# dlwns147/amq

Measured on AMD Instinct MI355X. Metric: decode tokens/s, Llama-2-7B AMQ mixed 2/3/4-bit avg-3-bit, batch 1, higher is better.
Workload: dtype f16; 1 GPU; Llama-2-7B shapes, synthesized avg-3.0-bit per-layer arch (bits_usage 2.982), batch 1 decode after a 64-token prefill, one stream per GPU; parallelism=replicas x1, prompt=64, group_size=128

## Files before the change

amq_amd/_lib.py:

```python
import ctypes
import os

_HERE = os.path.dirname(os.path.abspath(__file__))
LIB_PATH = os.path.join(_HERE, "libamq_hip.so")
AB_LIB_PATH = os.path.join(_HERE, "libamq_hip_ab.so")

AMQ_OK = 0
MODE_HQQ, MODE_FMA, MODE_FMA1 = 0, 1, 2
PRO_NONE, PRO_RMSNORM, PRO_SILU_MUL = 0, 1, 2
PRO_MUL = 4
MAX_SEGMENTS = 4
MATH_DEFAULT, MATH_LINEAR, MATH_GROUPSCALE, MATH_EXACT = 0, 1, 2, 3
FEWROW_AUTO, FEWROW_TILE, FEWROW_STREAM = 0, 1, 2
ABI_VERSION = 521
LOOKUP_STATE_WORDS = 32
STEP_STATE_STRIDE = 272
GEMM_AUTO, GEMM_TILED, GEMM_SKINNY, GEMM_RING, GEMM_RING128, GEMM_WS, GEMM_DEQ = 0, 1, 2, 3, 4, 5, 6
HQQ_ITERS = 20
HQQ_INFO_BYTES = 88
GPTQ_INFO_BYTES = 4
AWQ_INFO_BYTES = 4
OWQ_INFO_BYTES = 4
AWQ_STEPS = 10

_vp, _i, _f, _sz = ctypes.c_void_p, ctypes.c_int, ctypes.c_float, ctypes.c_size_t


class Segment(ctypes.Structure):
    _fields_ = [("qweight_native", _vp), ("meta_native", _vp), ("bias", _vp), ("residual", _vp),
                ("y", _vp), ("N", _i), ("bits", _i), ("mode", _i), ("y_stride", _i)]


class EngineLinear(ctypes.Structure):
    _fields_ = [("qweight_native", _vp), ("meta_native", _vp), ("N", _i), ("bits", _i), ("mode", _i), ("reserved", _i)]
# ... 77 lines not shown
    "amq_attn_prefill_xfrag_f16": (_i, [_vp, _vp, _vp, _vp, _i, _i, _i, _i, _i] + [ctypes.c_longlong] * 5 + [_vp]),
    "amq_gemv_f16w_rows": (_i, [_vp, _vp, _vp, _vp, _vp, _f, _i, _i, _i, _vp]),
    "amq_decode_tail_batch_f16": (_i, [_vp, _i, _vp, _i, _vp, _vp, _vp, _vp, _vp, _i, _i, _vp]),
    "amq_decode_tail_suppress_f16": (_i, [_vp, _i, _vp, _i, _vp, _vp, _vp, _vp, _vp, _i, _i, _vp, _vp]),
    "amq_sample_f16": (_i, [_vp, _i, _i, _vp, _vp, _vp, _vp, _vp, _i, _i, _vp]),
    "amq_decode_tail_sample_f16": (_i, [_vp, _i, _vp, _i, _vp, _vp, _vp, _vp, _vp, _i, _i, _vp, _vp, _vp]),
    "amq_logit_nll_f16": (_i, [_vp, ctypes.c_longlong, _vp, _i, _i, _vp, _vp, _vp, _vp]),
    "amq_logit_jsd_f16": (_i, [_vp, ctypes.c_longlong, _vp, ctypes.c_longlong, _i, _i, _i, _f, _vp, _vp]),
    "amq_set_token_f16": (_i, [_vp, _i, _vp, _i, _i, _vp, _vp, _vp, _vp, _vp, _i, _i, _vp]),
    "amq_attn_decode_seq_f16": (_i, [_vp, _vp, _vp, _vp, _vp, _vp, _vp, _i, _i, _i, _i, _i, _i, _vp, _sz, _vp, _vp]),
    "amq_decode_tail_seq_f16": (_i, [_vp, _i, _vp, _i, _vp, _vp, _vp, _vp, _i, _i, _vp, _vp]),
    "amq_decode_tail_sample_seq_f16": (_i, [_vp, _i, _vp, _i, _vp, _vp, _vp, _vp, _i, _i, _vp, _vp, _vp]),
    "amq_set_token_seq_f16": (_i, [_vp, _i, _vp, _i, _i, _vp, _vp, _vp, _vp, _i, _i, _vp]),
    "amq_attn_decode_rows_f16": (_i, [_vp, _vp, _vp, _vp, _vp, _vp, _vp, _i, _i, _i, _i, _i, _i, _vp, _sz, _vp, _vp]),
    "amq_attn_decode_rows_gqa_f16": (_i, [_vp, _vp, _vp, _vp, _vp, _vp, _vp, _i, _i, _i, _i, _i, _i, _vp, _sz, _vp, _vp]),
    "amq_decode_tail_lookup_f16": (_i, [_vp, _i, _vp, _i, _vp, _vp, _vp, _vp, _i, _i, _vp, _vp, _vp, _i, _vp]),
    "amq_decode_tail_lookup_sample_f16": (_i, [_vp, _i, _vp, _i, _vp, _vp, _vp, _vp, _i, _i, _vp, _vp, _vp, _i, _vp, _vp, _vp, _vp]),
    "amq_attn_prefill_f16": (_i, [_vp, _vp, _vp, _vp, _i, _i, _i, _i, _i, _i] + [ctypes.c_longlong] * 10 + [_vp]),
    "amq_rope_cache_f16": (_i, [_vp, _vp, _vp, _vp, _vp, _vp, _i, _i, _i, _i, _i, _i, _i, _vp]),
    "amq_rope_cache_batch_f16": (_i, [_vp, _vp, _vp, _vp, _vp, _vp, _i, _i, _i, _i, _i, _i, _i, _i, _vp]),
    "amq_rope_rows_f16": (_i, [_vp, _vp, _vp, _i, _i, _i, _i, _i, _i, _i, _vp]),
    "amq_silu_mul_f16": (_i, [_vp, _vp, _vp, _sz, _vp]),
    "amq_gemv_grouped_f16": (_i, [ctypes.POINTER(Segment), _i, _vp, _vp, _vp, _f, _i, _i, _i, _i, _i, ctypes.POINTER(GemvOpts), _vp]),
    "amq_gemv_grouped_sums_f16": (_i, [ctypes.POINTER(Segment), _i, _vp, _vp, _f, _vp, _vp, _i, _i, _i, _vp]),
    "amq_gemm_f16w_f16": (_i, [_vp, _vp, _vp, _vp, _vp, _vp, _i, _i, _i, _i, _i, _vp]),
    "amq_gemm_route_workspace_bytes": (_sz, [_i, _i, _i, _i]),
    "amq_gemm_route_workspace_bytes_g": (_sz, [_i, _i, _i, _i, _i]),
    "amq_gemm_res_norm_xfrag_f16": (_i, [_i, _i, _vp, _vp, _vp, _vp, _vp, _vp, _i, _i, _i, _i, _i, _vp, _sz, _vp, _f, _vp, _vp]),
    "amq_gemm_route_f16": (_i, [_i, _i, _i, _vp, _vp, _vp, _vp, _vp, _vp, _i, _i, _i, _i, _i, _i, _vp, _sz, _vp]),
}

for _base in ("amq_attn_decode_f16", "amq_attn_decode_cur_f16", "amq_attn_decode_split_f16", "amq_attn_decode_seq_f16", "amq_attn_decode_rows_f16",
              "amq_attn_decode_rows_gqa_f16",
              "amq_rope_cache_batch_f16", "amq_rope_rows_f16"):
    SIGNATURES[_base.replace("_batch", "")[:-len("_f16")] + "_qkn_f16"] = (_i, [_qkn] + SIGNATURES[_base][1])
del _base

AB_SIGNATURES = {
    "amq_gemv_qkv_attn_f16": (_i, [ctypes.POINTER(Segment), _vp, _vp, _f, _i, _i, _vp, _vp, _vp, _vp, _i, _i, _i, _i, _vp, _vp]),
    "amq_decode_engine_image_bytes": (_sz, [_i]),
    "amq_decode_engine_scratch_bytes": (_sz, [_i, _i, _i]),
    "amq_decode_engine_sync_bytes": (_sz, []),
    "amq_decode_engine_image": (_i, [ctypes.POINTER(EngineBlock), _i, _i, _i, _i, _i, _i, _i, _vp]),
    "amq_decode_engine_f16": (_i, [_vp, _i, _i, _i, _i, _i, _i, _i, _f, _vp, _vp, _sz, _vp, _vp, _sz, _i, _vp]),
}

# ... 122 lines not shown
```

amq_amd/csrc/amq_capi.hip:

```cpp
#include "../../include/amq_hip.h"
#ifdef AMQ_AB_ROUTES
#include "../../include/amq_hip_ab.h"
#endif
#include "amq_common.cuh"
#include "amq_kernels.h"

#include <stdarg.h>
#include <stdio.h>
#include <vector>

namespace {

thread_local char g_err[512] = "";

int fail(int code, const char* fmt, ...) {
    va_list ap;
    va_start(ap, fmt);
    vsnprintf(g_err, sizeof(g_err), fmt, ap);
    va_end(ap);
    return code;
}

int check_hip(hipError_t e, const char* what) {
    if (e == hipSuccess) return AMQ_OK;
// ... 268 lines not shown
}

#ifndef AMQ_GEMV_DEFAULT_MATH
#define AMQ_GEMV_DEFAULT_MATH AMQ_MATH_EXACT
#endif
int amq_default_gemv_math(void) { return AMQ_GEMV_DEFAULT_MATH; }

int amq_gemv_grouped_f16(const amq_segment* segs, int nseg, const void* x, const void* x2, const void* gamma,
                         float eps, int prologue, int M, int K, int group, int x_stride, const amq_gemv_opts* opts,
                         void* stream) {
    if (!segs || nseg < 1 || nseg > AMQ_MAX_SEGMENTS) return fail(AMQ_EINVAL, "nseg must be 1..%d (got %d)", AMQ_MAX_SEGMENTS, nseg);
    if (!x) return fail(AMQ_EINVAL, "null x");
    if ((prologue < AMQ_PRO_NONE || prologue > AMQ_PRO_SILU_MUL) && prologue != AMQ_PRO_MUL) return fail(AMQ_EINVAL, "unknown prologue %d", prologue);
    if (prologue == AMQ_PRO_RMSNORM && !gamma) return fail(AMQ_EINVAL, "RMSNorm prologue needs gamma");
    if (prologue == AMQ_PRO_SILU_MUL && !x2) return fail(AMQ_EINVAL, "SiLU*mul prologue needs x2");
    if (prologue == AMQ_PRO_MUL && !x2) return fail(AMQ_EINVAL, "mul prologue needs x2");
    if (M < 1) return fail(AMQ_ESHAPE, "M must be >= 1 (got %d)", M);
    amq_gemv_opts o{};
    if (opts) o = *opts;
    if (o.math < AMQ_MATH_DEFAULT || o.math > AMQ_MATH_EXACT)
        return fail(AMQ_EINVAL, "opts.math must be AMQ_MATH_DEFAULT, AMQ_MATH_EXACT, AMQ_MATH_GROUPSCALE or AMQ_MATH_LINEAR");
    if (o.math == AMQ_MATH_DEFAULT) o.math = amq_default_gemv_math();
    if (o.waves != 0 && o.waves != 4 && o.waves != 8 && o.waves != 16) return fail(AMQ_EINVAL, "opts.waves must be 0, 4, 8 or 16");
    if (o.depth != 0 && o.depth != 2 && o.depth != 4) return fail(AMQ_EINVAL, "opts.depth must be 0, 2 or 4");
    if (o.rpt < 0 || o.rpt > 64) return fail(AMQ_EINVAL, "opts.rpt (row-tiles per workgroup) must be 0..64");
    if (o.act_mask < 0 || o.act_mask >= (1 << nseg)) return fail(AMQ_EINVAL, "opts.act_mask names segments 0..%d (got 0x%x)", nseg - 1, o.act_mask);
    if ((o.act_mask || prologue == AMQ_PRO_MUL) && amq::meta_pairs(group) != 1)
        return fail(AMQ_ESHAPE, "opts.act_mask / AMQ_PRO_MUL: groups of 128 (and multiples) only (got %d); use AMQ_PRO_SILU_MUL", group);
    const bool plain_form = !o.dot && o.math != AMQ_MATH_LINEAR && o.depth != 4 && amq::meta_pairs(group) == 1 && o.waves != 4;
    const bool whole_rows = prologue == AMQ_PRO_RMSNORM || (x_stride != 0 && x_stride != K);
    if (M > amq::GEMV_MAX_M || amq::gemv_min_lds_bytes(M, K, plain_form && o.waves == 0 && o.rpt == 0, whole_rows) > LDS_LIMIT)
        return fail(AMQ_ESHAPE, "M=%d rows of K=%d%s do not fit LDS for the GEMV path; use amq_gemm_f16", M, K, (x_stride != 0 && x_stride != K) ? " (strided x)" : "");
    amq::GemvArgs a{};
    for (int i = 0; i < nseg; ++i) {
        const amq_segment& s = segs[i];
        if (int rc = check_shape(s.bits, s.N, K, group)) return rc;
        if (int rc = check_mode(s.mode)) return rc;
        if (!s.qweight_native || !s.meta_native || !s.y) return fail(AMQ_EINVAL, "segment %d: null pointer", i);
        amq::GemvSeg& d = a.seg[i];
        d.qweight = s.qweight_native; d.meta = s.meta_native; d.bias = s.bias; d.residual = s.residual; d.y = s.y;
        d.N = s.N; d.bits = s.bits; d.mode = s.mode;
        d.y_stride = s.y_stride ? s.y_stride : s.N;
        d.act = (o.act_mask >> i) & 1;
        if (d.act && s.residual) return fail(AMQ_EINVAL, "segment %d: an activated output (opts.act_mask) takes no residual", i);
    }
    a.nseg = nseg; a.M = M; a.K = K; a.x_stride = x_stride ? x_stride : K;
    a.x = x; a.x2 = x2; a.gamma = gamma; a.eps = eps; a.prologue = prologue;
    a.flags = (o.dot ? amq::GEMV_FLAG_DOT : 0) | (o.math == AMQ_MATH_LINEAR ? amq::GEMV_FLAG_LINEAR : 0) |
              (o.math == AMQ_MATH_GROUPSCALE ? amq::GEMV_FLAG_GS : 0);
    a.force_waves = o.waves;
    a.force_depth = o.depth;
    a.force_rpt = o.rpt;
    a.gp = amq::meta_pairs(group);
    if (a.gp > 1 && (o.dot || o.math == AMQ_MATH_LINEAR || o.depth == 4))
        return fail(AMQ_EINVAL, "groups of %d: the GEMV kernel's default form only (opts.math = AMQ_MATH_EXACT, opts.dot = 0, opts.depth = 0 / 2)", group);
    return check_hip(amq::launch_gemv(a, (hipStream_t)stream), "gemv");
}

int amq_gemv_grouped_sums_f16(const amq_segment* segs, int nseg, const void* x, const void* gamma, float eps, const float* sums_in,
                              float* sums_out, int M, int K, int group, void* stream) {
    if (!segs || nseg < 1 || nseg > AMQ_MAX_SEGMENTS) return fail(AMQ_EINVAL, "nseg must be 1..%d (got %d)", AMQ_MAX_SEGMENTS, nseg);
    if (!x) return fail(AMQ_EINVAL, "null x");
    if ((sums_in != nullptr) != (gamma != nullptr)) return fail(AMQ_EINVAL, "sums_in (the partial sums of squares of x) and gamma go together");
    if (M < 2 || M > 8) return fail(AMQ_ESHAPE, "the partial-sum forms live in the 2 .. 8-row kernels (got M=%d); one row: amq_gemv_grouped_f16 with AMQ_PRO_RMSNORM", M);
    if (amq::meta_pairs(group) != 1) return fail(AMQ_ESHAPE, "groups of 128 (and multiples) only (got %d)", group);
    if (K < 2048) return fail(AMQ_ESHAPE, "K >= 2048 (the 2 .. 8-row kernels run 8 or 16 waves per workgroup; got K=%d)", K);
    if (sums_out && nseg != 1) return fail(AMQ_EINVAL, "sums_out describes ONE output: nseg must be 1");
    if (sums_out && sums_in) return fail(AMQ_EINVAL, "sums_out is written by launches without a prologue (o_proj, down_proj): not together with sums_in");
    if (sums_in && K > 8192) return fail(AMQ_ESHAPE, "sums_in: K <= 8192 (K / 16 <= 512 partials per row; got K=%d)", K);
    const bool phased = amq::gemv_rows_phased(M, K, true, sums_in != nullptr);
    if (sums_in && phased) return fail(AMQ_ESHAPE, "M=%d rows of K=%d are staged in two K phases: no fused norm there", M, K);
    if (amq::gemv_min_lds_bytes(M, K, true, sums_in != nullptr) > LDS_LIMIT)
        return fail(AMQ_ESHAPE, "M=%d rows of K=%d do not fit LDS for the GEMV path", M, K);
    amq::GemvArgs a{};
    for (int i = 0; i < nseg; ++i) {
        const amq_segment& s = segs[i];
        if (int rc = check_shape(s.bits, s.N, K, group)) return rc;
        if (int rc = check_mode(s.mode)) return rc;
        if (!s.qweight_native || !s.meta_native || !s.y) return fail(AMQ_EINVAL, "segment %d: null pointer", i);
// ... 915 lines not shown
```

amq_amd/csrc/amq_gemv.hip:

```cpp
#include "amq_gemv_body.cuh"

namespace amq {


#ifdef AMQ_STAMP
unsigned long long* g_stamp_ptr = nullptr;
extern "C" int amq_debug_set_stamps(void* p) { g_stamp_ptr = (unsigned long long*)p; return 0; }
#endif

size_t gemv_lds_bytes(int M, int K, int nw) {
    const size_t xbytes = (((size_t)M * (K + XPAD) * 2) + 15) & ~(size_t)15;
    const size_t xg = (size_t)(K >> 7) * 64;
    const size_t red = (size_t)2 * (nw > 1 ? nw : 16) * 16 * 16 * 4;
    return xbytes + xg + red;
}

size_t gemv_lds_bytes_rows(int M, int K, int nw) {
    const size_t xbytes = (((size_t)M * (K + XPAD) * 2) + 15) & ~(size_t)15;
    return xbytes + (size_t)2 * nw * (M <= 4 ? 64 : 128) * 4;
}
bool gemv_rows_phased(int M, int K, bool plain, bool norm) {
    const int G = K >> 7;
    return plain && !norm && M > 4 && M <= 8 && (G & 1) == 0 && G / 2 >= 2 * 16 && (K / 2 >> 3) <= 1024 &&
           gemv_lds_bytes_rows(M, K, 16) > 160 * 1024 && gemv_lds_bytes_rows(M, K / 2, 16) <= 160 * 1024;
// ... 2 lines not shown
    if (gemv_rows_phased(M, K, plain, norm)) return gemv_lds_bytes_rows(M, K / 2, 16);
    if (plain && M > 1 && M <= 8) return gemv_lds_bytes_rows(M, K, 16);
    return gemv_lds_bytes(M, K, 1);
}

int gemv_pick_waves(int total_rt, int K) {
    const int G = K >> 7;
    if (G < 16) return 4;
    if (G > 32) return 16;
    return 8;
}

#define AMQ_GEMV_EXTERN(PRO_)                                                                                                  \
    extern template hipError_t launch_pro<PRO_>(const GemvKArgs&, int, int, int, int, size_t, hipStream_t);                     \
    extern template hipError_t launch_pro_g<PRO_, 2>(const GemvKArgs&, int, int, size_t, hipStream_t);                          \
    extern template hipError_t launch_pro_g<PRO_, 4>(const GemvKArgs&, int, int, size_t, hipStream_t);
AMQ_GEMV_EXTERN(PRO_NONE)
AMQ_GEMV_EXTERN(PRO_RMSNORM)
AMQ_GEMV_EXTERN(PRO_SILU_MUL)
#undef AMQ_GEMV_EXTERN
extern template hipError_t launch_pro<PRO_MUL>(const GemvKArgs&, int, int, int, int, size_t, hipStream_t);
hipError_t launch_pro_sums_entry(const GemvKArgs&, int nw, int rs, int, size_t, hipStream_t);

#ifndef AMQ_RS128_THREE
#define AMQ_RS128_THREE 1
#endif
hipError_t launch_gemv(GemvArgs& a, hipStream_t st) {
    StreamDevice sd_(st);
    int total_rt = 0;
    for (int i = 0; i < a.nseg; ++i) { a.seg[i].n_rt = a.seg[i].N / 16; total_rt += a.seg[i].n_rt; }
    int nw = a.force_waves ? a.force_waves : gemv_pick_waves(total_rt, a.K);
    const int gp = a.gp > 1 ? a.gp : 1;
    if (gp != 1 && gp != 2 && gp != 4) return hipErrorInvalidValue;
    if (gp > 1 && ((a.flags & (GEMV_FLAG_DOT | GEMV_FLAG_LINEAR)) || a.force_depth == 4)) return hipErrorInvalidValue;
    bool rs128 = false, rs64 = false;
    const bool plain = !(a.flags & (GEMV_FLAG_DOT | GEMV_FLAG_LINEAR)) && a.force_depth != 4 && gp == 1;
    const bool ph2 = !a.force_waves && a.force_rpt <= 0 && gemv_rows_phased(a.M, a.K, plain, a.prologue == PRO_RMSNORM || a.x_stride != a.K);
    if (ph2) {
        rs128 = true;
        nw = 16;
    } else if (a.M > 1 && a.M <= 8 && plain && nw != 4) {
        rs128 = a.M > 4;
        rs64 = !rs128;
        if (!a.force_waves && nw == 8 && 2 * gemv_lds_bytes_rows(a.M, a.K, 8) > 160 * 1024) nw = 16;
    } else if (!a.force_waves && a.M > 1 && nw == 8 && 3 * gemv_lds_bytes(a.M, a.K, 8) > 160 * 1024) {
        nw = 16;
    }
    const bool mid_k = gp == 1 && !a.force_waves && nw == 16 && a.M == 1 && (a.K >> 3) > 512 && (a.K >> 3) <= 1024 &&
                       !(a.flags & (GEMV_FLAG_DOT | GEMV_FLAG_LINEAR)) && a.force_depth != 4;
    if (mid_k) nw = 8;
    int rpt = ph2 ? 1 : a.force_rpt;
// ... 40 lines not shown
        k.wg_begin[i] = s.wg_begin; k.n_rt[i] = gemv_split(s.n_rt, s.wg_count); k.key[i] = s.bits * 4 + (s.mode == MODE_FMA1 && !has_fma1 ? (int)MODE_FMA : s.mode);
        k.qweight[i] = s.qweight; k.meta[i] = s.meta;
        k.bias[i] = s.bias; k.residual[i] = s.residual; k.y[i] = s.y; k.y_stride[i] = s.y_stride;
        k.act_mask |= (s.act ? 1 : 0) << i;
    }
#ifdef AMQ_STAMP
    k.stamps = g_stamp_ptr;
#endif
    if (gp == 2) {
        switch (a.prologue) {
            case PRO_NONE: return launch_pro_g<PRO_NONE, 2>(k, nw, wg, lds, st);
            case PRO_RMSNORM: return launch_pro_g<PRO_RMSNORM, 2>(k, nw, wg, lds, st);
            default: return launch_pro_g<PRO_SILU_MUL, 2>(k, nw, wg, lds, st);
        }
    }
    if (gp == 4) {
        switch (a.prologue) {
            case PRO_NONE: return launch_pro_g<PRO_NONE, 4>(k, nw, wg, lds, st);
            case PRO_RMSNORM: return launch_pro_g<PRO_RMSNORM, 4>(k, nw, wg, lds, st);
            default: return launch_pro_g<PRO_SILU_MUL, 4>(k, nw, wg, lds, st);
        }
    }
    if (a.prologue == PRO_RMSNORM_SUMS) return launch_pro_sums_entry(k, nw, rs64 ? 64 : 128, wg, lds, st);
    switch (a.prologue) {
        case PRO_NONE: return launch_pro<PRO_NONE>(k, a.flags | (rs128 ? GEMV_FLAG_RS128 : 0) | (rs64 ? GEMV_FLAG_RS64 : 0) | (ph2 ? GEMV_FLAG_PH2 : 0), a.force_depth, nw, wg, lds, st);
        case PRO_RMSNORM: return launch_pro<PRO_RMSNORM>(k, a.flags | (rs128 ? GEMV_FLAG_RS128 : 0) | (rs64 ? GEMV_FLAG_RS64 : 0) | (ph2 ? GEMV_FLAG_PH2 : 0), a.force_depth, nw, wg, lds, st);
        case PRO_MUL: return launch_pro<PRO_MUL>(k, a.flags | (rs128 ? GEMV_FLAG_RS128 : 0) | (rs64 ? GEMV_FLAG_RS64 : 0) | (ph2 ? GEMV_FLAG_PH2 : 0), a.force_depth, nw, wg, lds, st);
        default: return launch_pro<PRO_SILU_MUL>(k, a.flags | (rs128 ? GEMV_FLAG_RS128 : 0) | (rs64 ? GEMV_FLAG_RS64 : 0) | (ph2 ? GEMV_FLAG_PH2 : 0), a.force_depth, nw, wg, lds, st);
    }
}

}
```

amq_amd/csrc/amq_gemv_body.cuh:

```cuda
#pragma once
#include "amq_common.cuh"
#include "amq_kernels.h"

namespace amq {

constexpr int XPAD = 8;

struct GemvKArgs {
    const void* x; const void* x2; const void* gamma;
    int M, K, x_stride, nseg;
    float eps; int rpt, pad0_, pad1_;
    int wg_begin[GEMV_MAX_SEG];
    int n_rt[GEMV_MAX_SEG];
    int key[GEMV_MAX_SEG];
    const void* qweight[GEMV_MAX_SEG];
    const void* meta[GEMV_MAX_SEG];
    const void* bias[GEMV_MAX_SEG];
    const void* residual[GEMV_MAX_SEG];
    void* y[GEMV_MAX_SEG];
    int y_stride[GEMV_MAX_SEG];
    float* sums_out;
    int sums_stride;
    int act_mask;
#ifdef AMQ_STAMP
// ... 845 lines not shown
    const _Float16* xuse = xl;
    constexpr bool HAS_FMA1 = (MATH == MATH_EXACT || MATH == MATH_GS) && GP == 1;
    bool done = false;
    if constexpr (HAS_FMA1) {
        if (key == 4 * 4 + MODE_FMA1) { gemv_body<4, MODE_FMA1, PRO, NW, U, MATH, XCH, RS, false, GP, PH>(a, blk, sidx, qwp, mtp, nrt, local, xl, xuse, xg, red, xs, xmode, xr); done = true; }
        else if (key == 3 * 4 + MODE_FMA1) { gemv_body<3, MODE_FMA1, PRO, NW, U, MATH, XCH, RS, false, GP, PH>(a, blk, sidx, qwp, mtp, nrt, local, xl, xuse, xg, red, xs, xmode, xr); done = true; }
        else if (key == 2 * 4 + MODE_FMA1) { gemv_body<2, MODE_FMA1, PRO, NW, U, MATH, XCH, RS, false, GP, PH>(a, blk, sidx, qwp, mtp, nrt, local, xl, xuse, xg, red, xs, xmode, xr); done = true; }
    }
    if (!done) switch (key) {
        case 4 * 4 + MODE_HQQ: gemv_body<4, MODE_HQQ, PRO, NW, U, MATH, XCH, RS, false, GP, PH>(a, blk, sidx, qwp, mtp, nrt, local, xl, xuse, xg, red, xs, xmode, xr); break;
        case 3 * 4 + MODE_HQQ: gemv_body<3, MODE_HQQ, PRO, NW, U, MATH, XCH, RS, false, GP, PH>(a, blk, sidx, qwp, mtp, nrt, local, xl, xuse, xg, red, xs, xmode, xr); break;
        case 2 * 4 + MODE_HQQ: gemv_body<2, MODE_HQQ, PRO, NW, U, MATH, XCH, RS, false, GP, PH>(a, blk, sidx, qwp, mtp, nrt, local, xl, xuse, xg, red, xs, xmode, xr); break;
        case 4 * 4 + MODE_FMA: gemv_body<4, MODE_FMA, PRO, NW, U, MATH, XCH, RS, false, GP, PH>(a, blk, sidx, qwp, mtp, nrt, local, xl, xuse, xg, red, xs, xmode, xr); break;
        case 3 * 4 + MODE_FMA: gemv_body<3, MODE_FMA, PRO, NW, U, MATH, XCH, RS, false, GP, PH>(a, blk, sidx, qwp, mtp, nrt, local, xl, xuse, xg, red, xs, xmode, xr); break;
        default:               gemv_body<2, MODE_FMA, PRO, NW, U, MATH, XCH, RS, false, GP, PH>(a, blk, sidx, qwp, mtp, nrt, local, xl, xuse, xg, red, xs, xmode, xr); break;
    }
    if (threadIdx.x < 64) AMQ_STAMP_AT(blk, 4);
#ifdef AMQ_STAMP
    if (threadIdx.x == 0 && blk.stamps) blk.stamps[(size_t)blockIdx.x * 128 + 6] = __builtin_amdgcn_s_memtime();
#endif
}


template <int PRO, int NW, int U, int MATH, int XCH = XCfg<NW>::XC, int RS = 256, int GP = 1, int PH = 1>
inline hipError_t launch_one(const GemvKArgs& a, int total_wg, size_t lds, hipStream_t st) {
    auto kern = gemv_kernel<PRO, NW, U, MATH, XCH, RS, GP, PH>;
    if (lds > 64 * 1024) {
        hipError_t e = hipFuncSetAttribute((const void*)kern, hipFuncAttributeMaxDynamicSharedMemorySize, (int)lds);
        if (e != hipSuccess) return e;
    }
    const void* xw = PRO_X2<PRO> ? a.x2 : a.gamma;
    hipLaunchKernelGGL(kern, dim3(total_wg), dim3(NW * 64), lds, st, a.x, xw, a.qweight[0], a.meta[0], a.K,
                       a.M | ((a.x_stride == a.K ? 1 : 0) << 8) | (a.nseg << 16), a.rpt, a.n_rt[0], a.key[0], a.eps, a);
    return hipGetLastError();
}

template <int PRO, int NW, int MATH>
inline hipError_t launch_std(const GemvKArgs& a, int flags, int total_wg, size_t lds, hipStream_t st) {
    if (NW == 8 && (flags & GEMV_FLAG_RS64)) return launch_one<PRO, 8, 2, MATH, XCfg<8>::XC, 64>(a, total_wg, lds, st);
    if (NW == 8 && (flags & GEMV_FLAG_RS128)) return launch_one<PRO, 8, 2, MATH, XCfg<8>::XC, 128>(a, total_wg, lds, st);
    if (NW == 16 && (flags & GEMV_FLAG_RS64)) return launch_one<PRO, 16, 2, MATH, XCfg<16>::XC, 64>(a, total_wg, lds, st);
    if constexpr (NW == 16 && PRO != PRO_RMSNORM) {
        if (flags & GEMV_FLAG_PH2) return launch_one<PRO, 16, 2, MATH, 1, 128, 1, 2>(a, total_wg, lds, st);
    }
    if (NW == 16 && (flags & GEMV_FLAG_RS128)) return launch_one<PRO, 16, 2, MATH, XCfg<16>::XC, 128>(a, total_wg, lds, st);
    if (NW == 16 && a.M == 1 && (a.K >> 3) > XCfg<16>::XC * 1024 && (a.K >> 3) <= 4 * 1024)
// ... 37 lines not shown
```

amq_amd/csrc/amq_kernels.h:

```cpp
#pragma once
#include <hip/hip_runtime.h>
#include <stddef.h>
#include <stdint.h>

namespace amq {

inline hipError_t ensure_dyn_lds(unsigned long long& done_mask, const void* fn, int bytes) {
    int dev = 0;
    hipError_t e = hipGetDevice(&dev);
    if (e != hipSuccess) return e;
    const unsigned long long bit = 1ull << (dev & 63);
    if (__atomic_load_n(&done_mask, __ATOMIC_RELAXED) & bit) return hipSuccess;
    e = hipFuncSetAttribute(fn, hipFuncAttributeMaxDynamicSharedMemorySize, bytes);
    if (e == hipSuccess) __atomic_fetch_or(&done_mask, bit, __ATOMIC_RELAXED);
    return e;
}

struct StreamDevice {
    int prev = -1;
    bool switched = false;
    explicit StreamDevice(hipStream_t st) {
        hipDevice_t dev = 0;
        if (st == nullptr || hipGetDevice(&prev) != hipSuccess || hipStreamGetDevice(st, &dev) != hipSuccess) return;
        if ((int)dev != prev && hipSetDevice((int)dev) == hipSuccess) switched = true;
// ... 22 lines not shown
    int wg_count;
    int n_rt;
    int y_stride;
    int act;
};

struct GemvArgs {
    GemvSeg seg[GEMV_MAX_SEG];
    int nseg;
    int M, K;
    int x_stride;
    const void* x;
    const void* x2;
    const void* gamma;
    float eps;
    int prologue;
    int flags;
    int force_waves;
    int force_depth;
    int force_rpt;
    int gp;
    const void* sums_in;
    void* sums_out;
};
constexpr int GEMV_SPLIT_BASE_BITS = 12, GEMV_SPLIT_BASE_MASK = (1 << GEMV_SPLIT_BASE_BITS) - 1;
inline int gemv_split(int n_rt, int wg_count) { return (n_rt / wg_count) | ((n_rt % wg_count) << GEMV_SPLIT_BASE_BITS); }
enum { GEMV_FLAG_DOT = 1, GEMV_FLAG_LINEAR = 2, GEMV_FLAG_RS128 = 4 ,
       GEMV_FLAG_GS = 8 ,
       GEMV_FLAG_RS64 = 16 ,
       GEMV_FLAG_PH2 = 32  };
constexpr int GEMV_MAX_M = 16;

size_t gemv_lds_bytes(int M, int K, int copies);
size_t gemv_lds_bytes_rows(int M, int K, int nw);
size_t gemv_min_lds_bytes(int M, int K, bool plain, bool norm = true);
bool gemv_rows_phased(int M, int K, bool plain, bool norm);
hipError_t launch_gemv(GemvArgs& a, hipStream_t st);

struct GemmArgs {
    const void* x; const void* qweight; const void* meta; const void* bias; void* y;
    int M, N, K, bits, mode, x_stride, y_stride;
    float* ws;
    int splits;
    const void* residual;
    const void* gate;
    void* w16;
    int gp;
};
enum { GEMM_ROUTE_AUTO = 0, GEMM_ROUTE_TILED = 1, GEMM_ROUTE_SKINNY = 2, GEMM_ROUTE_RING = 3, GEMM_ROUTE_RING128 = 4, GEMM_ROUTE_WS = 5,
       GEMM_ROUTE_DEQ = 6  };
struct GemmNorm { const void* gamma; float eps; void* xf; bool done; };
hipError_t launch_gemm(const GemmArgs& a, hipStream_t st, int route = GEMM_ROUTE_AUTO, GemmNorm* norm = nullptr);
bool gemm_gate_fused(const GemmArgs& a, int route);
hipError_t launch_gemm_ring(const GemmArgs& a, hipStream_t st, int bm = 0);
bool gemm_ring_ok(const GemmArgs& a);
hipError_t launch_gemm_ws(const GemmArgs& a, hipStream_t st);
int gemm_ring_rows(int M, int N);
int gemm_many_rows_plan(int M, int N);
bool gemm_takes_ring(int M, int N, int K);
hipError_t launch_gemm_xfrag(const GemmArgs& a, hipStream_t st);
// ... 214 lines not shown
```

amq_amd/ops.py:

```python
import ctypes
import os

import torch

from . import _lib
from ._lib import (MODE_HQQ, MODE_FMA, MODE_FMA1, PRO_NONE, PRO_RMSNORM, PRO_SILU_MUL, Segment, GemvOpts, EngineBlock, EngineLinear,
                   GEMM_AUTO, GEMM_TILED, GEMM_SKINNY, GEMM_RING, GEMM_RING128, GEMM_WS, GEMM_DEQ, MATH_DEFAULT, MATH_EXACT, MATH_LINEAR, MATH_GROUPSCALE)

GROUP = 128


def _need(t, dtype, name, numel=None):
    if not isinstance(t, torch.Tensor) or not t.is_cuda:
        raise ValueError(f"{name}: expected a tensor on the GPU")
    if t.dtype != dtype:
        raise ValueError(f"{name}: expected {dtype}, got {t.dtype}")
    if not t.is_contiguous():
        raise ValueError(f"{name}: must be contiguous")
    if numel is not None and t.numel() != numel:
        raise ValueError(f"{name}: expected {numel} elements, got {t.numel()}")


FINE_GROUPS = (64, 32)

# ... 929 lines not shown
        arr[i] = Segment(_lib.ptr(s["qn"]), _lib.ptr(s["mn"]), _lib.ptr(s.get("bias")), _lib.ptr(s.get("residual")),
                         _lib.ptr(s["y"]), s["N"], s["bits"], s["mode"], 0)
    if prologue == PRO_RMSNORM:
        _need(gamma, torch.float16, "gamma", K)
    if x_activated and prologue != PRO_SILU_MUL:
        raise ValueError("x_activated goes with prologue=PRO_SILU_MUL")
    if prologue == PRO_SILU_MUL:
        x2 = _prep_x(x2, K)
        if x2.shape[0] != M:
            raise ValueError("x2 rows != x rows")
        if x_activated:
            prologue = _lib.PRO_MUL
    if opts is None:
        opts = DEFAULT_GEMV_OPTS
    act_mask = sum(1 << i for i, s in enumerate(segments) if s.get("act"))
    if act_mask:
        o = opts
        opts = GemvOpts(act_mask=act_mask) if o is None else GemvOpts(math=o.math, waves=o.waves, depth=o.depth, rpt=o.rpt, dot=o.dot, act_mask=act_mask)
    _lib.check(_lib.load().amq_gemv_grouped_f16(arr, len(segments), _lib.ptr(xx), _lib.ptr(x2), _lib.ptr(gamma),
                                                ctypes.c_float(eps), prologue, M, K, group, 0,
                                                ctypes.byref(opts) if opts is not None else None, _lib.current_stream()))


def gemv_grouped_sums(x, segments, K, gamma=None, eps=0.0, sums_in=None, sums_out=None):
    xx = _prep_x(x, K)
    M = xx.shape[0]
    if not 1 <= len(segments) <= _lib.MAX_SEGMENTS:
        raise ValueError(f"1..{_lib.MAX_SEGMENTS} segments")
    if any(s.get("act") for s in segments):
        raise ValueError("an activated segment (act) is a gate, not a hidden state: the partial-sum launches take none (gemv_grouped)")
    arr = (Segment * len(segments))()
    for i, s in enumerate(segments):
        _check_shape(s["bits"], s["N"], K)
        _check_native(s["qn"], s["mn"], s["bits"], s["N"], K)
        _need(s["y"], torch.float16, "y", M * s["N"])
        if s.get("bias") is not None:
            _need(s["bias"], torch.float16, "bias", s["N"])
        if s.get("residual") is not None:
            _need(s["residual"], torch.float16, "residual", M * s["N"])
        arr[i] = Segment(_lib.ptr(s["qn"]), _lib.ptr(s["mn"]), _lib.ptr(s.get("bias")), _lib.ptr(s.get("residual")),
                         _lib.ptr(s["y"]), s["N"], s["bits"], s["mode"], 0)
    if sums_in is not None:
        _need(gamma, torch.float16, "gamma", K)
        _need(sums_in, torch.float32, "sums_in", M * (K // 16))
    if sums_out is not None:
        _need(sums_out, torch.float32, "sums_out", M * (segments[0]["N"] // 16))
# ... 679 lines not shown
```

include/amq_hip.h:

```cpp
#ifndef AMQ_HIP_H
#define AMQ_HIP_H

#include <stddef.h>
#include <stdint.h>

#ifdef __cplusplus
extern "C" {
#endif

#define AMQ_VERSION 521

#define AMQ_OK            0
#define AMQ_EINVAL       -1
#define AMQ_ESHAPE       -2
#define AMQ_ELAUNCH      -3
#define AMQ_EUNSUPPORTED -4

#define AMQ_MODE_HQQ 0
#define AMQ_MODE_FMA 1
#define AMQ_MODE_FMA1 2

#define AMQ_PRO_NONE     0
#define AMQ_PRO_RMSNORM  1
#define AMQ_PRO_SILU_MUL 2
#define AMQ_PRO_MUL      4

#define AMQ_MAX_SEGMENTS 4

int amq_version(void);
const char* amq_last_error(void);

#define AMQ_MATH_DEFAULT    0
#define AMQ_MATH_LINEAR     1
#define AMQ_MATH_GROUPSCALE 2
#define AMQ_MATH_EXACT      3
int amq_default_gemv_math(void);

typedef struct amq_gemv_opts {
    int math;
    int waves;
    int depth;
    int rpt;
    int dot;
    int act_mask;
} amq_gemv_opts;

#define AMQ_GEMM_AUTO   0
#define AMQ_GEMM_TILED  1
#define AMQ_GEMM_SKINNY 2
#define AMQ_GEMM_RING   3
#define AMQ_GEMM_RING128 4
#define AMQ_GEMM_WS 5
#define AMQ_GEMM_DEQ 6

int amq_query(int K, int* out, int cap);

size_t amq_native_qweight_bytes(int bits, int N, int K);
float amq_fma1_scale_bound(int bits);
size_t amq_native_meta_bytes(int N, int K, int group);

int amq_repack_from_hqq(int bits, const void* W_q, const void* scale, const void* zero,
                        int N, int K, int group, void* qweight_native, void* meta_native, void* stream);
int amq_repack_from_gptq(int bits, const void* qweight, const void* scales, const void* zeros,
                         int N, int K, int group, void* qweight_native, void* meta_native, void* stream);
int amq_repack_from_awq(const void* qweight, const void* scales, const void* scaled_zeros,
                        int N, int K, int group, void* qweight_native, void* meta_native, void* stream);

#define AMQ_HQQ_INFO_BYTES 88
// ... 242 lines not shown
```

Measured before the change: 772.8 tokens/s.

## Add bit-width-keyed GEMV kernels specialized per segment bit combination

```diff
diff --git a/amq_amd/_lib.py b/amq_amd/_lib.py
--- a/amq_amd/_lib.py
+++ b/amq_amd/_lib.py
@@ -10,6 +10,8 @@
 PRO_NONE, PRO_RMSNORM, PRO_SILU_MUL = 0, 1, 2
 PRO_MUL = 4
 MAX_SEGMENTS = 4
+GEMV_ROUTE_GENERIC, GEMV_ROUTE_KEYED = 0, 1
+GEMV_DEPTH_GENERIC = -1
 MATH_DEFAULT, MATH_LINEAR, MATH_GROUPSCALE, MATH_EXACT = 0, 1, 2, 3
 FEWROW_AUTO, FEWROW_TILE, FEWROW_STREAM = 0, 1, 2
 ABI_VERSION = 521
@@ -133,6 +135,8 @@
     "amq_rope_rows_f16": (_i, [_vp, _vp, _vp, _i, _i, _i, _i, _i, _i, _i, _vp]),
     "amq_silu_mul_f16": (_i, [_vp, _vp, _vp, _sz, _vp]),
     "amq_gemv_grouped_f16": (_i, [ctypes.POINTER(Segment), _i, _vp, _vp, _vp, _f, _i, _i, _i, _i, _i, ctypes.POINTER(GemvOpts), _vp]),
+    "amq_gemv_route": (_i, [_i, _i, _i, _i, _i, ctypes.POINTER(_i), ctypes.POINTER(_i), ctypes.POINTER(GemvOpts)]),
+    "amq_gemv_segment_order": (_i, [_i, ctypes.POINTER(_i), _i, ctypes.POINTER(_i), ctypes.POINTER(_i)]),
     "amq_gemv_grouped_sums_f16": (_i, [ctypes.POINTER(Segment), _i, _vp, _vp, _f, _vp, _vp, _i, _i, _i, _vp]),
     "amq_gemm_f16w_f16": (_i, [_vp, _vp, _vp, _vp, _vp, _vp, _i, _i, _i, _i, _i, _vp]),
     "amq_gemm_route_workspace_bytes": (_sz, [_i, _i, _i, _i]),
diff --git a/amq_amd/csrc/amq_capi.hip b/amq_amd/csrc/amq_capi.hip
--- a/amq_amd/csrc/amq_capi.hip
+++ b/amq_amd/csrc/amq_capi.hip
@@ -314,7 +314,9 @@
         return fail(AMQ_EINVAL, "opts.math must be AMQ_MATH_DEFAULT, AMQ_MATH_EXACT, AMQ_MATH_GROUPSCALE or AMQ_MATH_LINEAR");
     if (o.math == AMQ_MATH_DEFAULT) o.math = amq_default_gemv_math();
     if (o.waves != 0 && o.waves != 4 && o.waves != 8 && o.waves != 16) return fail(AMQ_EINVAL, "opts.waves must be 0, 4, 8 or 16");
-    if (o.depth != 0 && o.depth != 2 && o.depth != 4) return fail(AMQ_EINVAL, "opts.depth must be 0, 2 or 4");
+    if (o.depth != 0 && o.depth != 2 && o.depth != 4 && o.depth != AMQ_GEMV_DEPTH_GENERIC) return fail(AMQ_EINVAL, "opts.depth must be 0, 2, 4 or AMQ_GEMV_DEPTH_GENERIC");
+    const bool generic = o.depth == AMQ_GEMV_DEPTH_GENERIC;
+    if (generic) o.depth = 0;
     if (o.rpt < 0 || o.rpt > 64) return fail(AMQ_EINVAL, "opts.rpt (row-tiles per workgroup) must be 0..64");
     if (o.act_mask < 0 || o.act_mask >= (1 << nseg)) return fail(AMQ_EINVAL, "opts.act_mask names segments 0..%d (got 0x%x)", nseg - 1, o.act_mask);
     if ((o.act_mask || prologue == AMQ_PRO_MUL) && amq::meta_pairs(group) != 1)
@@ -344,9 +346,33 @@
     a.force_depth = o.depth;
     a.force_rpt = o.rpt;
     a.gp = amq::meta_pairs(group);
+    a.generic = generic;
     if (a.gp > 1 && (o.dot || o.math == AMQ_MATH_LINEAR || o.depth == 4))
         return fail(AMQ_EINVAL, "groups of %d: the GEMV kernel's default form only (opts.math = AMQ_MATH_EXACT, opts.dot = 0, opts.depth = 0 / 2)", group);
     return check_hip(amq::launch_gemv(a, (hipStream_t)stream), "gemv");
+}
+
+static int gemv_flags_of(const amq_gemv_opts& o) {
+    const int math = o.math == AMQ_MATH_DEFAULT ? amq_default_gemv_math() : o.math;
+    return (o.dot ? amq::GEMV_FLAG_DOT : 0) | (math == AMQ_MATH_LINEAR ? amq::GEMV_FLAG_LINEAR : 0) | (math == AMQ_MATH_GROUPSCALE ? amq::GEMV_FLAG_GS : 0);
+}
+
+int amq_gemv_route(int prologue, int M, int K, int group, int nseg, const int* bits, const int* modes, const amq_gemv_opts* opts) {
+    if (!bits || !modes || nseg < 1 || nseg > AMQ_MAX_SEGMENTS) return fail(AMQ_EINVAL, "nseg must be 1..%d (got %d), bits and modes non-null", AMQ_MAX_SEGMENTS, nseg);
+    if (group != 32 && group != 64 && (group < 128 || group % 128 != 0)) return fail(AMQ_ESHAPE, "group must be 32, 64 or a multiple of 128 (got %d)", group);
+    amq_gemv_opts o{};
+    if (opts) o = *opts;
+    const bool generic = o.depth == AMQ_GEMV_DEPTH_GENERIC;
+    int km[AMQ_MAX_SEGMENTS];
+    for (int i = 0; i < nseg; ++i) km[i] = modes[i] == AMQ_MODE_HQQ ? (int)amq::MODE_HQQ : (int)amq::MODE_FMA;
+    return amq::gemv_route(prologue, M, K, amq::meta_pairs(group), nseg, bits, km, gemv_flags_of(o), o.waves, generic ? 0 : o.depth, o.rpt, generic);
+}
+
+int amq_gemv_segment_order(int nseg, const int* bits, int act_mask, int* order, int* act_mask_out) {
+    if (!bits || !order || nseg < 1 || nseg > AMQ_MAX_SEGMENTS) return fail(AMQ_EINVAL, "nseg must be 1..%d (got %d), bits and order non-null", AMQ_MAX_SEGMENTS, nseg);
+    const int m = amq::gemv_segment_order(nseg, bits, act_mask, order);
+    if (act_mask_out) *act_mask_out = m;
+    return AMQ_OK;
 }
 
 int amq_gemv_grouped_sums_f16(const amq_segment* segs, int nseg, const void* x, const void* gamma, float eps, const float* sums_in,
diff --git a/amq_amd/csrc/amq_gemv.hip b/amq_amd/csrc/amq_gemv.hip
--- a/amq_amd/csrc/amq_gemv.hip
+++ b/amq_amd/csrc/amq_gemv.hip
@@ -48,11 +48,50 @@
 extern template hipError_t launch_pro<PRO_MUL>(const GemvKArgs&, int, int, int, int, size_t, hipStream_t);
 hipError_t launch_pro_sums_entry(const GemvKArgs&, int nw, int rs, int, size_t, hipStream_t);
 
+bool gemv_keyed_geometry(int prologue, int M, int K, int gp, int nseg, const int* bits, const int* modes, int flags, int force_waves, int force_depth,
+                         int force_rpt) {
+    if (M != 1 || gp > 1 || flags != 0 || force_depth != 0 || force_rpt > 0 || nseg < 1 || K < 128) return false;
+    for (int i = 0; i < nseg; ++i)
+        if (modes[i] != MODE_HQQ || bits[i] < 2 || bits[i] > 4) return false;
+    int nw = force_waves ? force_waves : gemv_pick_waves(0, K);
+    if (!force_waves && nw == 16 && (K >> 3) > 512 && (K >> 3) <= 1024) nw = 8;
+    switch (prologue) {
+        case PRO_RMSNORM: return nw == 8 && (K >> 3) <= XCfg<8>::XC * 8 * 64 && nseg <= 3;
+        case PRO_NONE: return nw == 8 && (K >> 3) <= XCfg<8>::XC * 8 * 64 && nseg == 1;
+        case PRO_MUL:
+        case PRO_SILU_MUL: return nw == 16 && (K >> 3) <= XCfg<16>::XC * 16 * 64 && nseg == 1;
+    }
+    return false;
+}
+
+int gemv_segment_order(int nseg, const int* bits, int act_mask, int* order) {
+    int n = 0, mask = 0;
+    for (int b = 0; b <= 32 && n < nseg; ++b)
+        for (int i = 0; i < nseg; ++i)
+            if ((bits[i] < 0 ? 0 : bits[i] > 32 ? 32 : bits[i]) == b) {
+                mask |= ((act_mask >> i) & 1) << n;
+                order[n++] = i;
+            }
+    return mask;
+}
+
 #ifndef AMQ_RS128_THREE
 #define AMQ_RS128_THREE 1
 #endif
 hipError_t launch_gemv(GemvArgs& a, hipStream_t st) {
     StreamDevice sd_(st);
+    bool keyed_geo = false;
+    if (a.nseg >= 1 && a.nseg <= GEMV_MAX_SEG) {
+        int bits[GEMV_MAX_SEG], modes[GEMV_MAX_SEG], order[GEMV_MAX_SEG];
+        for (int i = 0; i < a.nseg; ++i) { bits[i] = a.seg[i].bits; modes[i] = a.seg[i].mode; }
+        keyed_geo = !a.sums_out && gemv_keyed_geometry(a.prologue, a.M, a.K, a.gp, a.nseg, bits, modes, a.flags, a.force_waves, a.force_depth, a.force_rpt);
+        if (keyed_geo) {
+            gemv_segment_order(a.nseg, bits, 0, order);
+            GemvSeg sorted[GEMV_MAX_SEG];
+            for (int i = 0; i < a.nseg; ++i) sorted[i] = a.seg[order[i]];
+            for (int i = 0; i < a.nseg; ++i) a.seg[i] = sorted[i];
+        }
+    }
     int total_rt = 0;
     for (int i = 0; i < a.nseg; ++i) { a.seg[i].n_rt = a.seg[i].N / 16; total_rt += a.seg[i].n_rt; }
     int nw = a.force_waves ? a.force_waves : gemv_pick_waves(total_rt, a.K);
@@ -139,6 +178,7 @@
         }
     }
     if (a.prologue == PRO_RMSNORM_SUMS) return launch_pro_sums_entry(k, nw, rs64 ? 64 : 128, wg, lds, st);
+    if (keyed_geo && !a.generic) return launch_keyed(k, a.prologue, wg, lds, st);
     switch (a.prologue) {
         case PRO_NONE: return launch_pro<PRO_NONE>(k, a.flags | (rs128 ? GEMV_FLAG_RS128 : 0) | (rs64 ? GEMV_FLAG_RS64 : 0) | (ph2 ? GEMV_FLAG_PH2 : 0), a.force_depth, nw, wg, lds, st);
         case PRO_RMSNORM: return launch_pro<PRO_RMSNORM>(k, a.flags | (rs128 ? GEMV_FLAG_RS128 : 0) | (rs64 ? GEMV_FLAG_RS64 : 0) | (ph2 ? GEMV_FLAG_PH2 : 0), a.force_depth, nw, wg, lds, st);
diff --git a/amq_amd/csrc/amq_gemv_body.cuh b/amq_amd/csrc/amq_gemv_body.cuh
--- a/amq_amd/csrc/amq_gemv_body.cuh
+++ b/amq_amd/csrc/amq_gemv_body.cuh
@@ -891,6 +891,119 @@
 }
 
 
+template <int PRO, int NW, int XCH, int KEY0, int KEY1, int KEY2>
+__global__ __launch_bounds__(NW * 64, AMQ_LB_WAVES_R(NW, 1, MATH_EXACT, XCH, 256)) void gemv_kernel_keyed(const void* p_x, const void* p_xw, const void* p_qw0,
+                                                                     const void* p_mt0, int p_K, int p_m_nseg, int p_rpt,
+                                                                     int p_n_rt0, int p_key0, float p_eps, GemvKArgs blk) {
+    static_assert(KEY0 >= 2 && KEY0 <= 4 && (KEY1 == 0 || (KEY1 >= KEY0 && KEY1 <= 4)) && (KEY2 == 0 || (KEY1 != 0 && KEY2 >= KEY1 && KEY2 <= 4)),
+                  "bit-widths in ascending order, absent segments last");
+    constexpr int NSEG = 1 + (KEY1 != 0) + (KEY2 != 0);
+    extern __shared__ __attribute__((aligned(16))) unsigned char smem[];
+#ifndef AMQ_NO_PRIO_PROGRESS
+    __builtin_amdgcn_s_setprio(3);
+#endif
+    GemvHot a;
+    a.x = p_x; a.x2 = p_xw; a.gamma = p_xw;
+    a.K = p_K; a.M = 1; a.rpt = p_rpt; a.eps = p_eps; a.x_stride = p_K;
+    const int xs = a.K + XPAD;
+    _Float16* xl = (_Float16*)smem;
+    const size_t xbytes = ((size_t)xs * 2 + 15) & ~(size_t)15;
+    float* red = (float*)(smem + xbytes);
+
+    XRegs xr;
+    int issue = 1;
+    asm volatile("" : "+s"(issue));
+    if (issue) x_issue<PRO, NW, XCH>(a, xr);
+
+    const int bid = (int)blockIdx.x;
+    int sidx = 0;
+    int wgb = 0, nrt = p_n_rt0;
+    const void* qwp = p_qw0;
+    const void* mtp = p_mt0;
+    if constexpr (NSEG > 1) {
+        if constexpr (NSEG == 2)
+            asm volatile("" ::"s"(blk.wg_begin[1]), "s"(blk.n_rt[1]), "s"(blk.qweight[1]), "s"(blk.meta[1]));
+        else
+            asm volatile("" ::"s"(blk.wg_begin[1]), "s"(blk.wg_begin[2]), "s"(blk.n_rt[1]), "s"(blk.n_rt[2]), "s"(blk.qweight[1]),
+                         "s"(blk.qweight[2]), "s"(blk.meta[1]), "s"(blk.meta[2]));
+#pragma unroll
+        for (int i = 1; i < NSEG; ++i) {
+            const bool take = bid >= blk.wg_begin[i];
+            sidx = take ? i : sidx;
+            wgb = take ? blk.wg_begin[i] : wgb;
+            nrt = take ? blk.n_rt[i] : nrt;
+            qwp = take ? blk.qweight[i] : qwp;
+            mtp = take ? blk.meta[i] : mtp;
+        }
+    }
+    const int local = bid - wgb;
+#define AMQ_KEYED_BODY(B_) gemv_body<B_, MODE_HQQ, PRO, NW, 2, MATH_EXACT, XCH>(a, blk, sidx, qwp, mtp, nrt, local, xl, xl, nullptr, red, xs, 1, xr)
+    if constexpr (NSEG == 1 || (KEY1 == KEY0 && (NSEG == 2 || KEY2 == KEY0))) {
+        AMQ_KEYED_BODY(KEY0);
+    } else if constexpr (NSEG == 2) {
+        if (sidx == 0) AMQ_KEYED_BODY(KEY0); else AMQ_KEYED_BODY(KEY1);
+    } else if constexpr (KEY1 == KEY0) {
+        if (sidx < 2) AMQ_KEYED_BODY(KEY0); else AMQ_KEYED_BODY(KEY2);
+    } else if constexpr (KEY2 == KEY1) {
+        if (sidx == 0) AMQ_KEYED_BODY(KEY0); else AMQ_KEYED_BODY(KEY1);
+    } else {
+        if (sidx == 0) AMQ_KEYED_BODY(KEY0); else if (sidx == 1) AMQ_KEYED_BODY(KEY1); else AMQ_KEYED_BODY(KEY2);
+    }
+#undef AMQ_KEYED_BODY
+}
+
+template <int PRO, int NW, int XCH, int KEY0, int KEY1 = 0, int KEY2 = 0>
+inline hipError_t launch_keyed_one(const GemvKArgs& a, int total_wg, size_t lds, hipStream_t st) {
+    auto kern = gemv_kernel_keyed<PRO, NW, XCH, KEY0, KEY1, KEY2>;
+    if (lds > 64 * 1024) {
+        hipError_t e = hipFuncSetAttribute((const void*)kern, hipFuncAttributeMaxDynamicSharedMemorySize, (int)lds);
+        if (e != hipSuccess) return e;
+    }
+    const void* xw = PRO_X2<PRO> ? a.x2 : a.gamma;
+    hipLaunchKernelGGL(kern, dim3(total_wg), dim3(NW * 64), lds, st, a.x, xw, a.qweight[0], a.meta[0], a.K,
+                       a.M | ((a.x_stride == a.K ? 1 : 0) << 8) | (a.nseg << 16), a.rpt, a.n_rt[0], a.key[0], a.eps, a);
+    return hipGetLastError();
+}
+template <int PRO, int NW, int XCH>
+inline hipError_t launch_keyed_1(const GemvKArgs& a, int total_wg, size_t lds, hipStream_t st) {
+    switch (a.key[0] >> 2) {
+        case 2: return launch_keyed_one<PRO, NW, XCH, 2>(a, total_wg, lds, st);
+        case 3: return launch_keyed_one<PRO, NW, XCH, 3>(a, total_wg, lds, st);
+        case 4: return launch_keyed_one<PRO, NW, XCH, 4>(a, total_wg, lds, st);
+    }
+    return hipErrorInvalidValue;
+}
+template <int PRO, int NW, int XCH>
+inline hipError_t launch_keyed_2(const GemvKArgs& a, int total_wg, size_t lds, hipStream_t st) {
+    switch ((a.key[0] >> 2) * 10 + (a.key[1] >> 2)) {
+        case 22: return launch_keyed_one<PRO, NW, XCH, 2, 2>(a, total_wg, lds, st);
+        case 23: return launch_keyed_one<PRO, NW, XCH, 2, 3>(a, total_wg, lds, st);
+        case 24: return launch_keyed_one<PRO, NW, XCH, 2, 4>(a, total_wg, lds, st);
+        case 33: return launch_keyed_one<PRO, NW, XCH, 3, 3>(a, total_wg, lds, st);
+        case 34: return launch_keyed_one<PRO, NW, XCH, 3, 4>(a, total_wg, lds, st);
+        case 44: return launch_keyed_one<PRO, NW, XCH, 4, 4>(a, total_wg, lds, st);
+    }
+    return hipErrorInvalidValue;
+}
+template <int PRO, int NW, int XCH>
+inline hipError_t launch_keyed_3(const GemvKArgs& a, int total_wg, size_t lds, hipStream_t st) {
+    switch ((a.key[0] >> 2) * 100 + (a.key[1] >> 2) * 10 + (a.key[2] >> 2)) {
+        case 222: return launch_keyed_one<PRO, NW, XCH, 2, 2, 2>(a, total_wg, lds, st);
+        case 223: return launch_keyed_one<PRO, NW, XCH, 2, 2, 3>(a, total_wg, lds, st);
+        case 224: return launch_keyed_one<PRO, NW, XCH, 2, 2, 4>(a, total_wg, lds, st);
+        case 233: return launch_keyed_one<PRO, NW, XCH, 2, 3, 3>(a, total_wg, lds, st);
+        case 234: return launch_keyed_one<PRO, NW, XCH, 2, 3, 4>(a, total_wg, lds, st);
+        case 244: return launch_keyed_one<PRO, NW, XCH, 2, 4, 4>(a, total_wg, lds, st);
+        case 333: return launch_keyed_one<PRO, NW, XCH, 3, 3, 3>(a, total_wg, lds, st);
+        case 334: return launch_keyed_one<PRO, NW, XCH, 3, 3, 4>(a, total_wg, lds, st);
+        case 344: return launch_keyed_one<PRO, NW, XCH, 3, 4, 4>(a, total_wg, lds, st);
+        case 444: return launch_keyed_one<PRO, NW, XCH, 4, 4, 4>(a, total_wg, lds, st);
+    }
+    return hipErrorInvalidValue;
+}
+hipError_t launch_keyed_qkv(const GemvKArgs& a, int total_wg, size_t lds, hipStream_t st);
+hipError_t launch_keyed(const GemvKArgs& a, int prologue, int total_wg, size_t lds, hipStream_t st);
+
 template <int PRO, int NW, int U, int MATH, int XCH = XCfg<NW>::XC, int RS = 256, int GP = 1, int PH = 1>
 inline hipError_t launch_one(const GemvKArgs& a, int total_wg, size_t lds, hipStream_t st) {
     auto kern = gemv_kernel<PRO, NW, U, MATH, XCH, RS, GP, PH>;
diff --git a/amq_amd/csrc/amq_gemv_keyed0.hip b/amq_amd/csrc/amq_gemv_keyed0.hip
--- /dev/null
+++ b/amq_amd/csrc/amq_gemv_keyed0.hip
@@ -0,0 +1,6 @@
+#include "amq_gemv_body.cuh"
+namespace amq {
+hipError_t launch_keyed_qkv(const GemvKArgs& a, int total_wg, size_t lds, hipStream_t st) {
+    return launch_keyed_3<PRO_RMSNORM, 8, XCfg<8>::XC>(a, total_wg, lds, st);
+}
+}
diff --git a/amq_amd/csrc/amq_gemv_keyed1.hip b/amq_amd/csrc/amq_gemv_keyed1.hip
--- /dev/null
+++ b/amq_amd/csrc/amq_gemv_keyed1.hip
@@ -0,0 +1,22 @@
+#include "amq_gemv_body.cuh"
+namespace amq {
+hipError_t launch_keyed(const GemvKArgs& a, int prologue, int total_wg, size_t lds, hipStream_t st) {
+    switch (prologue) {
+        case PRO_RMSNORM:
+            if (a.nseg == 3) return launch_keyed_qkv(a, total_wg, lds, st);
+            if (a.nseg == 2) return launch_keyed_2<PRO_RMSNORM, 8, XCfg<8>::XC>(a, total_wg, lds, st);
+            if (a.nseg == 1) return launch_keyed_1<PRO_RMSNORM, 8, XCfg<8>::XC>(a, total_wg, lds, st);
+            break;
+        case PRO_NONE:
+            if (a.nseg == 1) return launch_keyed_1<PRO_NONE, 8, XCfg<8>::XC>(a, total_wg, lds, st);
+            break;
+        case PRO_MUL:
+            if (a.nseg == 1) return launch_keyed_1<PRO_MUL, 16, XCfg<16>::XC>(a, total_wg, lds, st);
+            break;
+        case PRO_SILU_MUL:
+            if (a.nseg == 1) return launch_keyed_1<PRO_SILU_MUL, 16, XCfg<16>::XC>(a, total_wg, lds, st);
+            break;
+    }
+    return hipErrorInvalidValue;
+}
+}
diff --git a/amq_amd/csrc/amq_kernels.h b/amq_amd/csrc/amq_kernels.h
--- a/amq_amd/csrc/amq_kernels.h
+++ b/amq_amd/csrc/amq_kernels.h
@@ -68,6 +68,7 @@
     int gp;
     const void* sums_in;
     void* sums_out;
+    int generic;
 };
 constexpr int GEMV_SPLIT_BASE_BITS = 12, GEMV_SPLIT_BASE_MASK = (1 << GEMV_SPLIT_BASE_BITS) - 1;
 inline int gemv_split(int n_rt, int wg_count) { return (n_rt / wg_count) | ((n_rt % wg_count) << GEMV_SPLIT_BASE_BITS); }
@@ -82,6 +83,14 @@
 size_t gemv_min_lds_bytes(int M, int K, bool plain, bool norm = true);
 bool gemv_rows_phased(int M, int K, bool plain, bool norm);
 hipError_t launch_gemv(GemvArgs& a, hipStream_t st);
+enum { GEMV_ROUTE_GENERIC = 0, GEMV_ROUTE_KEYED = 1 };
+bool gemv_keyed_geometry(int prologue, int M, int K, int gp, int nseg, const int* bits, const int* modes, int flags, int force_waves, int force_depth,
+                         int force_rpt);
+inline int gemv_route(int prologue, int M, int K, int gp, int nseg, const int* bits, const int* modes, int flags, int force_waves, int force_depth,
+                      int force_rpt, bool generic) {
+    return !generic && gemv_keyed_geometry(prologue, M, K, gp, nseg, bits, modes, flags, force_waves, force_depth, force_rpt) ? GEMV_ROUTE_KEYED : GEMV_ROUTE_GENERIC;
+}
+int gemv_segment_order(int nseg, const int* bits, int act_mask, int* order);
 
 struct GemmArgs {
     const void* x; const void* qweight; const void* meta; const void* bias; void* y;
diff --git a/amq_amd/ops.py b/amq_amd/ops.py
--- a/amq_amd/ops.py
+++ b/amq_amd/ops.py
@@ -975,6 +975,22 @@
                                                 ctypes.byref(opts) if opts is not None else None, _lib.current_stream()))
 
 
+def gemv_route(prologue, M, K, bits, modes=None, group=GROUP, opts=None):
+    n = len(bits)
+    modes = [MODE_HQQ] * n if modes is None else list(modes)
+    rc = _lib.load().amq_gemv_route(prologue, M, K, group, n, (ctypes.c_int * n)(*bits), (ctypes.c_int * n)(*modes),
+                                    ctypes.byref(opts) if opts is not None else None)
+    _lib.check(min(rc, 0))
+    return rc
+
+
+def gemv_segment_order(bits, act_mask=0):
+    n = len(bits)
+    order, mask = (ctypes.c_int * n)(), ctypes.c_int(0)
+    _lib.check(_lib.load().amq_gemv_segment_order(n, (ctypes.c_int * n)(*bits), act_mask, order, ctypes.byref(mask)))
+    return list(order), mask.value
+
+
 def gemv_grouped_sums(x, segments, K, gamma=None, eps=0.0, sums_in=None, sums_out=None):
     xx = _prep_x(x, K)
     M = xx.shape[0]
diff --git a/include/amq_hip.h b/include/amq_hip.h
--- a/include/amq_hip.h
+++ b/include/amq_hip.h
@@ -44,6 +44,13 @@
     int dot;
     int act_mask;
 } amq_gemv_opts;
+#define AMQ_GEMV_DEPTH_GENERIC (-1)
+
+#define AMQ_GEMV_ROUTE_GENERIC 0
+#define AMQ_GEMV_ROUTE_KEYED   1
+int amq_gemv_route(int prologue, int M, int K, int group, int nseg, const int* bits , const int* modes ,
+                   const amq_gemv_opts* opts );
+int amq_gemv_segment_order(int nseg, const int* bits , int act_mask, int* order , int* act_mask_out);
 
 #define AMQ_GEMM_AUTO   0
 #define AMQ_GEMM_TILED  1
```

Result: faster. 799.0 tokens/s (median of 6 runs) (+3.4%).
